# pzou1974/foremast-1

Measured on AMD Instinct MI355X. Metric: metric-series scored/sec (whole node) + p50 detect latency, 100k-series canary, higher is better.
Workload: dtype bf16

## Files before the change

### foremast_amd/ops/csrc/hw_scan.hip

```cpp
#include "common.h"
#include "detect.h"
#include "args.h"

#include <cstdlib>
#include <type_traits>

extern __shared__ __attribute__((aligned(16))) char fm_hw_smem[];

namespace {

enum { MODE_ES = 0, MODE_DES = 1, MODE_HW = 2 };

template <int CTRL, int RM>
__device__ __forceinline__ float dppf(float old, float src) {
  return __int_as_float(__builtin_amdgcn_update_dpp(__float_as_int(old), __float_as_int(src), CTRL, RM, 0xf, false));
}
template <int CTRL, int RM>
__device__ __forceinline__ v2f dpp2(float old, v2f src) {
  v2f r;
  r.x = dppf<CTRL, RM>(old, src.x);
  r.y = dppf<CTRL, RM>(old, src.y);
  return r;
}
__device__ __forceinline__ float rdlane(float v, int l) {
// ... 364 lines not shown
  v2f r;
  r.x = __int_as_float(__builtin_amdgcn_mov_dpp(__float_as_int(src.x), CTRL, RM, 0xf, true));
  r.y = __int_as_float(__builtin_amdgcn_mov_dpp(__float_as_int(src.y), CTRL, RM, 0xf, true));
  return r;
}
template <int CTRL>
__device__ __forceinline__ void row_round_z(v2f& w1, v2f& w2, const Mat2& Bd) {
  const v2f q1 = dppz2<CTRL, 0xf>(w1);
  const v2f q2 = dppz2<CTRL, 0xf>(w2);
  w1 = w1 + Bd.a * q1 + Bd.b * q2;
  w2 = w2 + Bd.c * q1 + Bd.d * q2;
}
__device__ __forceinline__ void half_uniform_scan_pre(const Mat2* Bp, cfp tab_b, v2f v1, v2f v2, v2f x01, v2f x02,
                                                      const Mat2& Bj, bool odd_row, v2f& s1, v2f& s2) {
  const Mat2 B16 = ldmat(tab_b + 32);
  v2f w1 = dppz2<0x111, 0xf>(v1);
  v2f w2 = dppz2<0x111, 0xf>(v2);
  row_round_z<0x111>(w1, w2, Bp[0]);
  row_round_z<0x112>(w1, w2, Bp[1]);
  row_round_z<0x114>(w1, w2, Bp[2]);
  row_round_z<0x118>(w1, w2, Bp[3]);
  v2f e1, e2;
  matvec(Bp[0], w1, w2, e1, e2);
  e1 = e1 + v1;
  e2 = e2 + v2;
  const v2f E1 = dppz2<0x142, 0xa>(e1), E2 = dppz2<0x142, 0xa>(e2);
  v2f y1, y2;
  matvec(B16, x01, x02, y1, y2);
  y1 = odd_row ? y1 + E1 : x01;
  y2 = odd_row ? y2 + E2 : x02;
  matvec(Bj, y1, y2, s1, s2);
  s1 = s1 + w1;
  s2 = s2 + w2;
}

__device__ __forceinline__ void row_uniform_scan_pre(const Mat2* Bp, v2f v1, v2f v2, v2f x01, v2f x02,
                                                     const Mat2& Bj, v2f& s1, v2f& s2) {
  v2f w1 = dppz2<0x111, 0xf>(v1);
  v2f w2 = dppz2<0x111, 0xf>(v2);
  row_round_z<0x111>(w1, w2, Bp[0]);
  row_round_z<0x112>(w1, w2, Bp[1]);
  row_round_z<0x114>(w1, w2, Bp[2]);
  row_round_z<0x118>(w1, w2, Bp[3]);
  matvec(Bj, x01, x02, s1, s2);
  s1 = s1 + w1;
  s2 = s2 + w2;
}

template <typename V>
__device__ __forceinline__ void half_exclusive_scan(Aff<V>& a, int j) {
  scan_round<0x111, 0xf>(a);
  scan_round<0x112, 0xf>(a);
  scan_round<0x114, 0xf>(a);
  scan_round<0x118, 0xf>(a);
  scan_round<0x142, 0xa>(a);
  a.m11 = dppv<0x138, 0xf>(1.f, a.m11);
  a.m12 = dppv<0x138, 0xf>(0.f, a.m12);
  a.m21 = dppv<0x138, 0xf>(0.f, a.m21);
  a.m22 = dppv<0x138, 0xf>(1.f, a.m22);
  a.v1 = dppv<0x138, 0xf>(0.f, a.v1);
  a.v2 = dppv<0x138, 0xf>(0.f, a.v2);
  if (j == 0) {
    const V one = splatv<V>(1.f), zero = splatv<V>(0.f);
    a.m11 = one; a.m12 = zero; a.m21 = zero; a.m22 = one; a.v1 = zero; a.v2 = zero;
  }
}
// ... 344 lines not shown
      "v_add_f32_dpp %0, %0, %0 row_bcast:15 row_mask:0xa bank_mask:0xf\n"
      "v_add_f32_dpp %1, %1, %1 row_bcast:15 row_mask:0xa bank_mask:0xf\n"
      "s_nop 1"
      : "+v"(v.x), "+v"(v.y));
  return v;
}

__device__ __forceinline__ v2f row_sum_last(v2f v) {
  asm volatile(
      "s_nop 1\n"
      "v_add_f32_dpp %0, %0, %0 row_shr:1 row_mask:0xf bank_mask:0xf bound_ctrl:1\n"
      "v_add_f32_dpp %1, %1, %1 row_shr:1 row_mask:0xf bank_mask:0xf bound_ctrl:1\n"
      "s_nop 1\n"
      "v_add_f32_dpp %0, %0, %0 row_shr:2 row_mask:0xf bank_mask:0xf bound_ctrl:1\n"
      "v_add_f32_dpp %1, %1, %1 row_shr:2 row_mask:0xf bank_mask:0xf bound_ctrl:1\n"
      "s_nop 1\n"
      "v_add_f32_dpp %0, %0, %0 row_shr:4 row_mask:0xf bank_mask:0xf bound_ctrl:1\n"
      "v_add_f32_dpp %1, %1, %1 row_shr:4 row_mask:0xf bank_mask:0xf bound_ctrl:1\n"
      "s_nop 1\n"
      "v_add_f32_dpp %0, %0, %0 row_shr:8 row_mask:0xf bank_mask:0xf bound_ctrl:1\n"
      "v_add_f32_dpp %1, %1, %1 row_shr:8 row_mask:0xf bank_mask:0xf bound_ctrl:1\n"
      "s_nop 1"
      : "+v"(v.x), "+v"(v.y));
  return v;
}

template <int SEL>
__device__ __forceinline__ v2f pk_splat(v2f pair) {
  v2f r;
  if (SEL == 0) asm volatile("v_pk_mov_b32 %0, %1, %1 op_sel:[0,0]" : "=v"(r) : "v"(pair));
  else asm volatile("v_pk_mov_b32 %0, %1, %1 op_sel:[1,1]" : "=v"(r) : "v"(pair));
  return r;
}
template <int K, int R>
__device__ __forceinline__ void d_pass1_steps(int q, const Chunk8f& cc, const v2f* wc, v2f* D, v2f& p1, v2f& p2) {
  if constexpr (R < 8) {
    const int i = 8 * q + R;
    if (i < K) {
      D[i] = pk_splat<R & 1>(chunk_pair<R>(cc));
      p1 = p1 + wc[2 * R] * D[i];
      p2 = p2 + wc[2 * R + 1] * D[i];
    }
    d_pass1_steps<K, R + 1>(q, cc, wc, D, p1, p2);
  }
}

template <int K>
__device__ __forceinline__ void d_pass1(const float* blk, cfp W, v2f* D, v2f& p1, v2f& p2) {
  constexpr int NCH = (K + 7) / 8;
  p1 = splat2(0.f);
  p2 = splat2(0.f);
  Chunk8f cc, cn;
  cn.load(blk);
#pragma unroll
  for (int q = 0; q < NCH; ++q) {
    v2f wc[16];
    W = launder(W);
#pragma unroll
    for (int r = 0; r < 16; ++r)
      if (16 * q + r < 2 * K) wc[r] = ldv2(W + 32 * q + 2 * r);
    cc = cn;
    if (q + 1 < NCH) cn.load(blk + (q + 1) * D_CHUNK);
    fence_sched();
    d_pass1_steps<K, 0>(q, cc, wc, D, p1, p2);
    fence_sched();
  }
}

__device__ __forceinline__ v2f keep_if(v2f e, unsigned keep, int bit) {
  const int mk = ((int)(keep << (31 - bit))) >> 31;
  v2f r;
  r.x = __int_as_float(__float_as_int(e.x) & mk);
  r.y = __int_as_float(__float_as_int(e.y) & mk);
  return r;
}

template <int K, bool FUSE, int R, bool M2 = false, bool R1 = false, bool SAVE = false>
__device__ __forceinline__ void d_steps(int q, const Chunk8f& cc, v2f* D, v2f c1, v2f c2, v2f g1a, const v2f* wc,
                                        v2f& x1, v2f& x2, v2f& sse, v2f& p1, v2f& p2, unsigned k2 = 0u,
                                        unsigned k1 = 0u, v2f* E = nullptr) {
  if constexpr (R < 8) {
    const int i = 8 * q + R;
    if (i < K) {
      v2f e = D[i] - x1;
      if (M2) e = keep_if(e, k2, i & 31);
      if constexpr (SAVE) {
        if (i & 1) asm volatile("v_mov_b32 %0, %1" : "=v"(E[i >> 1].y) : "v"(e.x));
        else asm volatile("v_mov_b32 %0, %1" : "=v"(E[i >> 1].x) : "v"(e.x));
      }
      const v2f t = x1 + x2;
      x1 = t + c1 * e;
      x2 = x2 + c2 * e;
      sse = sse + e * e;
      if (FUSE) {
        D[i] = add_dy<R>(D[i], cc) - g1a * e;
        if (R1) {
          const v2f tz = p1 + p2;
          const v2f ez = keep_if(D[i] - p1, k1, i & 31);
          p1 = tz + c1 * ez;
          p2 = p2 + c2 * ez;
        } else {
          p1 = p1 + wc[2 * R] * D[i];
          p2 = p2 + wc[2 * R + 1] * D[i];
        }
      } else if (i < HALF_HB) {
        D[i] = D[i] - g1a * e;
      }
    }
    d_steps<K, FUSE, R + 1, M2, R1, SAVE>(q, cc, D, c1, c2, g1a, wc, x1, x2, sse, p1, p2, k2, k1, E);
  }
}

template <int K>
__device__ __forceinline__ void d_chunk0(const float* blk, cfp W, Chunk8f& c, v2f* w) {
  c.load(blk);
#pragma unroll
  for (int r = 0; r < 16; ++r)
    if (r < 2 * K) w[r] = ldv2(W + 2 * r);
}

template <int K, bool FUSE, bool M2 = false, bool R1 = false, int L = 32, bool SAVE = false>
__device__ __forceinline__ void d_pass2(const float* blk, v2f* D, v2f c1, v2f c2, v2f g1a, cfp W, v2f& x1,
                                        v2f& x2, v2f& sse, v2f& p1, v2f& p2, cfp tb = nullptr,
                                        Mat2* Bn = nullptr, bool chk = false, const unsigned* ubp = nullptr,
                                        int* alive = nullptr, const Chunk8f* c0 = nullptr, const v2f* w0 = nullptr,
                                        unsigned k2lo = 0u, unsigned k2hi = 0u, unsigned k1lo = 0u,
                                        unsigned k1hi = 0u, v2f* E = nullptr) {
  constexpr int NCH = (K + 7) / 8;
  constexpr bool WTS = FUSE && !R1;
  if (FUSE) { p1 = splat2(0.f); p2 = splat2(0.f); }
  fence_sched();
  Chunk8f cc, cn;
  v2f wc[16], wn[16];
  unsigned ub = 0x7f800000u;
  if (FUSE && chk) ub = __hip_atomic_load(ubp, __ATOMIC_RELAXED, __HIP_MEMORY_SCOPE_WORKGROUP);
  if (WTS) {
    if (c0) {
      cn = *c0;
#pragma unroll
      for (int r = 0; r < 16; ++r) wn[r] = w0[r];
    } else {
      d_chunk0<K>(blk, W, cn, wn);
    }
  } else if (FUSE) {
    cn.load(blk);
  }
#pragma unroll
  for (int q = 0; q < NCH; ++q) {
    if (FUSE && q + 1 == NCH && chk) {
      const v2f s = L == 32 ? half_sum_last(sse) : row_sum_last(sse);
      const float U = __uint_as_float(ub);
      int v = ((lane_id() & (L - 1)) == L - 1 && !(s.x > U && s.y > U)) ? 1 : 0;
      asm volatile("" : "+v"(v));
      *alive = v;
    }
    if (WTS) {
      cc = cn;
#pragma unroll
      for (int r = 0; r < 16; ++r) wc[r] = wn[r];
      asm volatile("" ::"v"(cc.lo.x), "v"(cc.hi.x), "s"(wc[0].x));
      if (q + 1 < NCH) {
        W = launder(W);
        cn.load(blk + (q + 1) * D_CHUNK);
#pragma unroll
        for (int r = 0; r < 16; ++r)
          if (16 * (q + 1) + r < 2 * K) wn[r] = ldv2(W + 32 * (q + 1) + 2 * r);
      } else if (Bn) {
        tb = launder(tb);
#pragma unroll
        for (int b = 0; b < 4; ++b) Bn[b] = ldmat(tb + 8 * b);
      }
    } else if (FUSE) {
      cc = cn;
      asm volatile("" ::"v"(cc.lo.x), "v"(cc.hi.x));
      if (q + 1 < NCH) cn.load(blk + (q + 1) * D_CHUNK);
    }
    fence_sched();
    d_steps<K, FUSE, 0, M2, R1, SAVE>(q, cc, D, c1, c2, g1a, wc, x1, x2, sse, p1, p2, q < 4 ? k2lo : k2hi,
                                      q < 4 ? k1lo : k1hi, E);
    fence_sched();
  }
  if (WTS && Bn) {
    asm volatile("" ::"s"(Bn[0].a.x), "s"(Bn[3].d.y));
    fence_sched();
  }
}

__device__ __forceinline__ int hint_pair_at(int k, int lo, unsigned hp) {
  const int h0 = (int)(hp & 0xffffu), h1 = (int)(hp >> 16);
  const int nh = (h0 != 0xffff) + (h1 != 0xffff);
  if (k < nh) return (k == 0 && h0 != 0xffff) ? h0 : h1;
  int r = lo + k - nh;
  const int a0 = h0 < h1 ? h0 : h1, a1 = h0 < h1 ? h1 : h0;
  r += r >= a0 ? 1 : 0;
  r += r >= a1 ? 1 : 0;
  return r;
}

constexpr int QUAD_ITEM = 0x10000;
struct QuadQueue {
  int h0, h1, nh, nq, n_items;
  bool sib;
  __device__ __forceinline__ QuadQueue(int lo, int hi, unsigned hp) {
    h0 = (int)(hp & 0xffffu);
    h1 = (int)(hp >> 16);
    if (h0 == 0xffff) { h0 = h1; h1 = 0xffff; }
    nh = (h0 != 0xffff) + (h1 != 0xffff);
    sib = nh == 2 && (h0 ^ 1) == h1;
    nq = ((hi - lo) >> 1) - (sib ? 1 : nh);
    n_items = nh + nq + (sib ? 0 : nh);
  }
  __device__ __forceinline__ int at(int k, int lo) const {
    if (k < nh) return k == 0 ? h0 : h1;
    k -= nh;
    if (k < nq) {
      int r = (lo >> 1) + k;
      const int q0 = h0 >> 1, q1 = sib ? 0x7fff : h1 >> 1;
      const int a0 = q0 < q1 ? q0 : q1, a1 = q0 < q1 ? q1 : q0;
      r += r >= a0 ? 1 : 0;
      r += r >= a1 ? 1 : 0;
      return (2 * r) | QUAD_ITEM;
    }
    return (k == nq ? h0 : h1) ^ 1;
  }
};

template <int K, int R>
__device__ __forceinline__ void d_replay_steps(int q, const Chunk8f& cd, const Chunk8f& cy, const v2f* wc,
                                               const v2f* E, v2f g1a, v2f* D, v2f& p1, v2f& p2) {
  if constexpr (R < 8) {
    const int i = 8 * q + R;
    if (i < K) {
      D[i] = pk_splat<R & 1>(chunk_pair<R>(cd));
      D[i] = add_dy<R>(D[i], cy) - g1a * pk_splat<R & 1>(E[i >> 1]);
      p1 = p1 + wc[2 * R] * D[i];
      p2 = p2 + wc[2 * R + 1] * D[i];
    }
    d_replay_steps<K, R + 1>(q, cd, cy, wc, E, g1a, D, p1, p2);
  }
}

template <int K>
__device__ __forceinline__ void d_replay(const float* blk, const float* dyb, cfp W, const v2f* E, v2f g1a, v2f* D,
                                         v2f& p1, v2f& p2) {
  constexpr int NCH = (K + 7) / 8;
  p1 = splat2(0.f);
  p2 = splat2(0.f);
  Chunk8f cd, cy;
#pragma unroll
  for (int q = 0; q < NCH; ++q) {
    v2f wc[16];
    W = launder(W);
#pragma unroll
    for (int r = 0; r < 16; ++r)
      if (16 * q + r < 2 * K) wc[r] = ldv2(W + 32 * q + 2 * r);
    cd.load(blk + q * D_CHUNK);
    cy.load(dyb + q * D_CHUNK);
    fence_sched();
    d_replay_steps<K, 0>(q, cd, cy, wc, E, g1a, D, p1, p2);
    fence_sched();
  }
}


template <int K, int S>
struct DLds {
  static constexpr int SEA = DLay<K>::SEASON;
  static constexpr int NMW = ((64 / S) * K + 31) / 32;
  static constexpr int ZEROED = S * NMW + 4 * S * D_WAVES + 4;
  static constexpr int QUEUE = S, HINTS = S + 1;
  static constexpr int UBOUND = (S + 2 + 3) & ~3;
  static constexpr int FIXED = ZEROED + S * HALF_HB + D_WAVES * S * HALF_HB + D_WAVES * S * 4 + UBOUND;
  __host__ __device__ static constexpr size_t words(int ns1) { return (size_t)S * ns1 * SEA + FIXED; }
  __host__ __device__ static constexpr size_t gap_words(int ns1) { return (size_t)2 * ns1 * 64 + 2 * ns1 + 2; }

  float* dl;
  unsigned* vmask;
  float* stat;
  int* flag;
  float* ylast;
  float* bests;
  float* wbest;
  unsigned* ubound;
  unsigned* mbits;
  int* segm;
  float* nvc;
  __device__ __forceinline__ explicit DLds(int ns1) {
    dl = (float*)fm_hw_smem;
    vmask = (unsigned*)(dl + (size_t)S * ns1 * SEA);
    stat = (float*)(vmask + S * NMW);
    flag = (int*)(stat + 4 * S * D_WAVES);
    ylast = (float*)(flag + 4);
// ... 330 lines not shown
      const int q = atomicAdd(deferred, 1);
      if (q < (a.N + 1) / 2) deferred[1 + q] = n0;
    }
    return;
  }
  d_lds_init(L, a, tid, n0, hints, pi_lo, pi_hi);
  const int head = a.head_dev ? *a.head_dev : a.head;
  __syncthreads();

  int bad = 0;
  d_stage<T>(L, a, n0, head, tid, lane, w, bad);
  if (bad) atomicOr(L.flag, 1);
  __syncthreads();
  if (*L.flag) {
    if (tid == 0 && hid == 0) {
      const int q = atomicAdd(deferred, 1);
      if (q < (a.N + 1) / 2) deferred[1 + q] = n0;
      gflags[n0 >> 1] = 1;
    }
    return;
  }
  float l0r[2], b0r[2];
  d_means(L, m, ns1, tid, l0r, b0r);
  __syncthreads();

  const float l0 = pick(l0r, half), b0 = pick(b0r, half);
  const float* mydl = L.dl + (size_t)half * ns1 * SEA + j * 4;
  const int last_addr = ((lane & 32) | 31) << 2;
  Best best = {__builtin_huge_valf(), 0x7fffffff, l0, b0};
  float* mybest = L.bests + (w * 2 + half) * HALF_HB;
  const int nwaves = blockDim.x / FM_WAVE;
  const int npb = pi_hi - pi_lo;
  const unsigned hints_pp = (unsigned)__builtin_amdgcn_readfirstlane((int)L.ubound[L.HINTS]);
  const bool quads = share && ns1 >= 2 && ((pi_lo | pi_hi) & 1) == 0;
  const QuadQueue qq(pi_lo, pi_hi, hints_pp);
  const int n_items = quads ? qq.n_items : npb;
  v2f D[K];
  v2f E[(K + 1) / 2];
  float sX1, sX2, ssse;
  constexpr int ALONE = 0, FIRST = 1, SECOND = 2;
  const auto walk = [&](auto mode, int pi) __attribute__((always_inline)) {
    constexpr int MODE = decltype(mode)::value;
    GridPair<K> gp(a, pi, lane);
    v2f X1, X2, sse, p1, p2;
    if constexpr (MODE == SECOND) {
      d_replay<K>(mydl, mydl + SEA, gp.W, E, gp.g1a, D, p1, p2);
      X1 = splat2(sX1); X2 = splat2(sX2); sse = splat2(ssse);
    } else {
      X1 = splat2(l0 + b0); X2 = splat2(b0); sse = splat2(0.f);
      d_pass1<K>(mydl, gp.W, D, p1, p2);
    }
    if constexpr (MODE == FIRST) {
      v2f x1, x2;
      Chunk8f c0;
      v2f w0[16];
      asm volatile("" : "+v"(sse));
      d_chunk0<K>(mydl + SEA, launder(gp.W), c0, w0);
      half_uniform_scan_pre(gp.Bp, launder(gp.tb), p1, p2, X1, X2, gp.Bj, odd_row, x1, x2);
      d_pass2<K, true, false, false, 32, true>(mydl + SEA, D, gp.c1, gp.c2, gp.g1a, launder(gp.W), x1, x2, sse, p1, p2,
                                               gp.tb, gp.Bp, false, nullptr, nullptr, &c0, w0, 0u, 0u, 0u, 0u, E);
      X1 = half_last_bp(x1, last_addr);
      X2 = half_last_bp(x2, last_addr);
      sX1 = X1.x; sX2 = X2.x; ssse = sse.x;
    }
    int alive = 1;
    for (int sg = MODE == ALONE ? 1 : 2; sg < nseg - 1; ++sg) {
      v2f x1, x2;
      Chunk8f c0;
      v2f w0[16];
      d_chunk0<K>(mydl + (size_t)sg * SEA, launder(gp.W), c0, w0);
      half_uniform_scan_pre(gp.Bp, launder(gp.tb), p1, p2, X1, X2, gp.Bj, odd_row, x1, x2);
      d_pass2<K, true>(mydl + (size_t)sg * SEA, D, gp.c1, gp.c2, gp.g1a, launder(gp.W), x1, x2, sse, p1, p2, gp.tb,
                       gp.Bp, PRUNE, L.ubound + half, &alive, &c0, w0);
      X1 = half_last_bp(x1, last_addr);
      X2 = half_last_bp(x2, last_addr);
      if (PRUNE && !__any(alive)) break;
    }
    if (!PRUNE || __any(alive)) {
      v2f x1, x2, d1, d2;
      half_uniform_scan_pre(gp.Bp, gp.tb, p1, p2, X1, X2, gp.Bj, odd_row, x1, x2);
      d_pass2<K, false>(mydl, D, gp.c1, gp.c2, gp.g1a, gp.W, x1, x2, sse, d1, d2);
      X1 = half_last_bp(x1, last_addr);
      X2 = half_last_bp(x2, last_addr);
      sse = half_sum_last(sse);
      sse = half_last_bp(sse, last_addr);
      take_candidate<PRUNE>(best, sse, X1, X2, gp.c0, gp.c1i, j == 0, L.ubound + half,
                            [&](bool upd1) __attribute__((always_inline)) {
        first_lane_phases<K>(mybest, L.ylast + half * HALF_HB, D, upd1, j, hmax);
      });
    }
  };
  for (int k = w; k < n_items;) {
    const int item = quads ? qq.at(k, pi_lo) : hint_pair_at(k, pi_lo, hints_pp);
    if (item & QUAD_ITEM) {
      walk(std::integral_constant<int, FIRST>(), item & 0xffff);
      walk(std::integral_constant<int, SECOND>(), (item & 0xffff) + 1);
    } else {
      walk(std::integral_constant<int, ALONE>(), item);
    }
    k = queue_pop(L.ubound + L.QUEUE, lane, nwaves);
  }

  if (j == 0) put_wave_best<2>(L.wbest, w, half, best);
  __syncthreads();
  if (w >= 2) return;
  const int r = w, n = n0 + r;
  if (n >= a.N) return;
  const int win = wave_argmin<2>(L.wbest, r, nwaves);
  const float* wb = L.wbest + (win * 2 + r) * 4;
  float gSSE = wb[0], gL = wb[2], gB = wb[3];
  int gIdx = __float_as_int(wb[1]);
  float* sb = L.bests + (win * 2 + r) * HALF_HB;
  if (slot >= 0) {
    float* mine = cand + (((size_t)slot * 2 + hid) * 2 + r) * CAND_FLOATS;
    if (lane < HALF_HB) __hip_atomic_store(&mine[4 + lane], sb[lane], __ATOMIC_RELAXED, __HIP_MEMORY_SCOPE_SYSTEM);
    if (lane == 0) {
      __hip_atomic_store(&mine[0], gSSE, __ATOMIC_RELAXED, __HIP_MEMORY_SCOPE_SYSTEM);
      __hip_atomic_store(&mine[1], __int_as_float(gIdx), __ATOMIC_RELAXED, __HIP_MEMORY_SCOPE_SYSTEM);
      __hip_atomic_store(&mine[2], gL, __ATOMIC_RELAXED, __HIP_MEMORY_SCOPE_SYSTEM);
      __hip_atomic_store(&mine[3], gB, __ATOMIC_RELAXED, __HIP_MEMORY_SCOPE_SYSTEM);
    }
    asm volatile("s_waitcnt vmcnt(0)" ::: "memory");
    int prev = 0;
    if (lane == 0) prev = __hip_atomic_fetch_add(&cnt[slot * 2 + r], 1, __ATOMIC_RELAXED, __HIP_MEMORY_SCOPE_AGENT);
    prev = __shfl(prev, 0, FM_WAVE);
    if (prev == 0) return;
    if (lane == 0) __hip_atomic_store(&cnt[slot * 2 + r], 0, __ATOMIC_RELAXED, __HIP_MEMORY_SCOPE_AGENT);
    const float* oth = cand + (((size_t)slot * 2 + (1 - hid)) * 2 + r) * CAND_FLOATS;
    const float oSSE = __hip_atomic_load(&oth[0], __ATOMIC_RELAXED, __HIP_MEMORY_SCOPE_SYSTEM);
    const int oIdx = __float_as_int(__hip_atomic_load(&oth[1], __ATOMIC_RELAXED, __HIP_MEMORY_SCOPE_AGENT));
    if (oSSE < gSSE || (oSSE == gSSE && oIdx < gIdx)) {
      gSSE = oSSE;
      gIdx = oIdx;
// ... 562 lines not shown
static bool d_supported_k(int K) { return K == 45 || K == 9; }
static bool q_supported_k(int K) { return K == 18; }

static size_t d_lds_words(int Tp, int seg, int K, bool gapped) {
  if (!d_supported_k(K) || seg <= 0) return (size_t)-1;
  const int nseg = Tp / seg;
  if (nseg < 2 || nseg > D_MAXSEG) return (size_t)-1;
  const int ns1 = nseg - 1;
  const size_t gap = gapped ? DLds<45, 2>::gap_words(ns1) : 0;
  return (K == 45 ? DLds<45, 2>::words(ns1) : DLds<9, 2>::words(ns1)) + gap;
}

extern "C" size_t fm_hw_d_lds_bytes(int Tp, int seg, int K) {
  const size_t words = d_lds_words(Tp, seg, K, false);
  return words == (size_t)-1 ? words : words * 4;
}

extern "C" size_t fm_hw_dg_lds_bytes(int Tp, int seg, int K) {
  const size_t words = d_lds_words(Tp, seg, K, true);
  return words == (size_t)-1 ? words : words * 4;
}

extern "C" size_t fm_hw_q_lds_bytes(int Tp, int seg, int K) {
  if (!q_supported_k(K) || seg != 16 * K) return (size_t)-1;
  const int nseg = Tp / seg;
  if (nseg < 2 || nseg > D_MAXSEG) return (size_t)-1;
  return DLds<18, Q_S>::words(nseg - 1) * 4;
}

struct GridSwitches {
  bool prune;
  int hints;
  int share;
};
static GridSwitches grid_switches() {
  const char* pe = getenv("FOREMAST_HW_PRUNE");
  const char* he = getenv("FOREMAST_HW_HINTS");
  const char* se = getenv("FOREMAST_HW_SHARE");
  GridSwitches s;
  s.prune = !(pe && pe[0] == '0');
  s.hints = (s.prune && !(he && he[0] == '0')) ? 1 : 0;
  s.share = !(se && se[0] == '0') ? 1 : 0;
  return s;
}

template <bool PRUNE, typename T>
static hipError_t launch_q_fit(const SmoothArgs* a, const float* tab_g, int hmax, int* deferred, int hints,
                               hipStream_t st) {
  const int K = a->K;
  const size_t lds = fm_hw_q_lds_bytes(a->Tp, a->seg, K);
  const size_t dlds = fm_hw_dg_lds_bytes(a->Tp, a->seg, K / 2);
  const int quads = (a->N + 3) / 4;
  hipLaunchKernelGGL((hw_q_kernel<18, PRUNE, T>), dim3(quads), dim3(256), lds, st, *a, hmax, deferred, hints);
  hipError_t e = hipGetLastError();
  if (e != hipSuccess) return e;
  SmoothArgs ag = *a;
  ag.pair_tab = tab_g;
  ag.K = K / 2;
  const int pairs = (a->N + 1) / 2;
  const int grid = pairs < 512 ? pairs : 512;
  hipLaunchKernelGGL((hw_dg_kernel<9, PRUNE, T>), dim3(grid), dim3(256), dlds, st, ag, hmax, deferred, hints);
  return hipGetLastError();
}

extern "C" int fm_hw_q_fit_dt(const SmoothArgs* a, const float* tab_g, int hmax, int* deferred, hipStream_t st,
                              int fp32) {
  const int K = a->K;
  if (!q_supported_k(K) || a->seg != 16 * K || a->m != a->seg || a->Tp % a->seg != 0 || a->Tp / a->seg < 2 ||
      a->Tp / a->seg > D_MAXSEG || !a->pair_tab || !tab_g || a->season_out || hmax < 1 || hmax > K ||
      hmax > HALF_HB)
    return (int)hipErrorNotSupported;
  if (a->N <= 0) return 0;
  if (fm_hw_q_lds_bytes(a->Tp, a->seg, K) > 80 * 1024 || fm_hw_dg_lds_bytes(a->Tp, a->seg, K / 2) > 80 * 1024)
    return (int)hipErrorNotSupported;
  if (!deferred) return (int)hipErrorInvalidValue;
// ... 93 lines not shown
  if (e != hipSuccess) return e;
  const char* ge = getenv("FOREMAST_HW_GAPS");
  if (K == 45 && std::is_same<T, bf16_t>::value && ge && ge[0] == 'v') {
    const size_t glds = fm_hw_half_lds_bytes(a->Tp, a->seg, K);
    if (glds > 64 * 1024) return hipErrorNotSupported;
    hipLaunchKernelGGL((hw_half_general_kernel<45>), dim3(pairs < 512 ? pairs : 512), dim3(256), glds, st, *a, hmax,
                       deferred);
    return hipGetLastError();
  }
  const size_t dlds = fm_hw_dg_lds_bytes(a->Tp, a->seg, K);
  int grid = pairs < 512 ? pairs : 512;
  const char* gg = getenv("FOREMAST_HW_DG_GRID");
  if (gg && atoi(gg) > 0) grid = atoi(gg) < pairs ? atoi(gg) : pairs;
  hipLaunchKernelGGL((hw_dg_kernel<K, PRUNE, T>), dim3(grid), dim3(256), dlds, st, *a, hmax, deferred, hints);
  return hipGetLastError();
}

extern "C" int fm_hw_d_fit_split_dt(const SmoothArgs* a, int hmax, int* deferred, int* split_ws, int max_split,
                                    int slots, hipStream_t st, int grid_quads, int fp32) {
  const int K = a->K;
  if (!d_supported_k(K) || a->seg != 32 * K || a->m != a->seg || a->Tp % a->seg != 0 || a->Tp / a->seg < 2 ||
      a->Tp / a->seg > D_MAXSEG || !a->pair_tab || a->season_out || hmax < 1 || hmax > K || hmax > HALF_HB)
    return (int)hipErrorNotSupported;
  if (a->N <= 0) return 0;
  if (fm_hw_d_lds_bytes(a->Tp, a->seg, K) > 80 * 1024 || fm_hw_dg_lds_bytes(a->Tp, a->seg, K) > 80 * 1024)
    return (int)hipErrorNotSupported;
  if (!deferred) return (int)hipErrorInvalidValue;
  const GridSwitches sw = grid_switches();
  const auto launch =
      fp32 ? (K == 45 ? (sw.prune ? launch_d_fit<45, true, float> : launch_d_fit<45, false, float>)
                      : (sw.prune ? launch_d_fit<9, true, float> : launch_d_fit<9, false, float>))
           : (K == 45 ? (sw.prune ? launch_d_fit<45, true, bf16_t> : launch_d_fit<45, false, bf16_t>)
                      : (sw.prune ? launch_d_fit<9, true, bf16_t> : launch_d_fit<9, false, bf16_t>));
  return (int)launch(a, hmax, deferred, split_ws, max_split, slots, sw.hints, (sw.share && grid_quads) ? 1 : 0, st);
}

extern "C" int fm_hw_d_fit_split(const SmoothArgs* a, int hmax, int* deferred, int* split_ws, int max_split,
                                 int slots, hipStream_t st, int grid_quads) {
  return fm_hw_d_fit_split_dt(a, hmax, deferred, split_ws, max_split, slots, st, grid_quads, 0);
}

extern "C" int fm_hw_d_fit(const SmoothArgs* a, int hmax, int* deferred, hipStream_t st) {
  return fm_hw_d_fit_split(a, hmax, deferred, nullptr, 0, 0, st, 0);
}

template <int K, int MODE, typename TIN, int NC, int MINW, bool TAB = false>
__global__ __launch_bounds__(256, MINW) void hw_scan_kernel(const SmoothArgs a) {
  static_assert(!TAB || NC == 2, "table path is packed-pair only");
  using V = typename std::conditional<NC == 2, v2f, float>::type;
  using YR = YRegs<TIN, K>;
  constexpr int KP = YR::KP;
  const int n = blockIdx.x;
  const int tid = threadIdx.x, lane = lane_id(), w = wave_id();
  const int nwaves = blockDim.x / FM_WAVE;
  const int seg = a.seg;
  const int L = seg / K;
  const int nseg = a.Tp / seg;

  size_t off = 0;
  TIN* ys = (TIN*)(fm_hw_smem + off);
  off += ((size_t)nseg * 64 * KP * sizeof(TIN) + 15) & ~(size_t)15;
  float* bests = (float*)(fm_hw_smem + off);
  if (MODE == MODE_HW) off += (size_t)nwaves * 64 * KP * 4;
  int* segnan = (int*)(fm_hw_smem + off);
  off += ((size_t)nseg * 4 + 15) & ~(size_t)15;
  float* red = (float*)(fm_hw_smem + off);
  off += 64 * 4;
// ... 300 lines not shown
```

### foremast_amd/ops/kernels.py

```python

from __future__ import annotations

import collections
import ctypes as C
import os
from dataclasses import dataclass
from typing import Tuple, Dict, Optional

import torch

from . import _native as nat

MODE_ES, MODE_DES, MODE_HW = 0, 1, 2
DEFAULT_ES_K = 16
LDS_LIMIT = 64 * 1024
D_LDS_LIMIT = 78 * 1024
LDS_MAX_WG = 160 * 1024


class KernelShapeError(ValueError):
    pass


def _need(cond: bool, msg: str) -> None:
# ... 257 lines not shown
            c1 = al + c2
            A = np.array([[1 - c1, 1.0], [-c2, 1.0]])
            Ap = np.eye(2)
            for n in range(K + 1):
                for q, v in enumerate((Ap[0, 0], Ap[0, 1], Ap[1, 0], Ap[1, 1])):
                    pw[p, n, 2 * q + comp] = v
                Ap = A @ Ap
    t = torch.tensor(np.concatenate([tab.reshape(-1), pw.reshape(-1)]), dtype=torch.float32,
                     device=grid.device).contiguous()
    if len(_PAIR_TAB_CACHE) > 64:
        _PAIR_TAB_CACHE.clear()
    _PAIR_TAB_CACHE[key] = t
    return t


_GRID_QUADS_CACHE: Dict[tuple, bool] = {}


def grid_has_quads(grid: torch.Tensor) -> bool:
    key = (grid.data_ptr(), tuple(grid.shape), grid.device)
    hit = _GRID_QUADS_CACHE.get(key)
    if hit is None:
        G = grid.shape[0]
        hit = False
        if G > 0 and G % 4 == 0 and grid.dim() == 2 and grid.shape[1] >= 2:
            ab = grid.detach()[:, :2].float().cpu().contiguous().view(torch.int32).view(G // 4, 4, 2)
            hit = bool((ab == ab[:, :1]).all())
        if len(_GRID_QUADS_CACHE) > 64:
            _GRID_QUADS_CACHE.clear()
        _GRID_QUADS_CACHE[key] = hit
    return hit


def smoothing_supported(mode: int, T: int, m: int, bf16: bool) -> bool:
    try:
        Tp, _, k, seg = smoothing_geometry(mode, T, m)
    except KernelShapeError:
        return False
    lib = nat.load()
    if lib is None:
        return False
    return lib.fm_smooth_lds_bytes(Tp, m if mode == MODE_HW else 1, seg, int(bf16)) <= LDS_LIMIT


def _fit_outputs(out: Optional[Dict[str, torch.Tensor]], N: int, dev, names, m: int = 0,
                 zeroed=()) -> Dict[str, torch.Tensor]:
    out = {} if out is None else out
    for name in names:
        if name not in out:
            shape = (N, HALF_HB) if name == "season_hb" else (N, m) if name == "season" else (N,)
            make = torch.zeros if name in zeroed else torch.empty
            out[name] = make(shape, dtype=torch.int32 if name == "best" else torch.float32, device=dev)
    return out


def _smooth_args(out: Dict[str, torch.Tensor], N: int, *, Tp: int, m: int, pad: int = 0, K: int = 0, seg: int = 0,
                 hist: Optional[torch.Tensor] = None, head: int = 0, length: int = 0,
                 grid: Optional[torch.Tensor] = None) -> "nat.SmoothArgs":
    a = nat.SmoothArgs()
    if hist is not None:
        a.hist = nat.ptr(hist)
        a.ld = hist.stride(0)
        a.ring_len = hist.shape[1]
        a.head = int(head)
        a.T = int(length)
    a.Tp, a.pad, a.m, a.K, a.seg = int(Tp), int(pad), int(m), int(K), int(seg)
# ... 133 lines not shown
    N = hist.shape[0]
    k = m // 16 if quad else m // 32
    out = _fit_outputs(out, N, dev, ("level", "trend", "sigma", "best") + (("season_hb", "nvalid") if defer else ()))
    a = _smooth_args(out, N, Tp=Tp, m=m, pad=pad, K=k, seg=m, hist=hist, head=head, length=length, grid=grid)
    a.pair_tab = nat.ptr(pair_table(grid, k))
    if head_dev is not None:
        _need(head_dev.dtype == torch.int32 and head_dev.device == dev and head_dev.numel() >= 1,
              "head_dev must be an int32 device scalar")
        a.head_dev = nat.ptr(head_dev)
    _fill_detect(a.det, det, N, dev, out)
    _set_hvar(a.det, det, grid, MODE_HW, m)
    if defer:
        a.season_hb = nat.ptr(out["season_hb"])
        a.nvalid_out = nat.ptr(out["nvalid"])
        a.det.C = 0
    ws = _half_workspace(dev, N)
    global last_hw_variant, last_detect_deferred
    last_detect_deferred = defer
    fp32 = int(hist.dtype == torch.float32)
    _need(residual or not fp32, "HW variant 4 needs a bfloat16 ring")
    if quad:
        rc = lib.fm_hw_q_fit_dt(a, nat.ptr(pair_table(grid, m // 32)), int(hmax), nat.ptr(ws),
                                nat.stream_handle(dev), fp32)
        if rc != 0:
            ws.zero_()
        nat.check(rc, "fm_hw_q_fit_dt")
        last_hw_variant = 5
        return out
    if residual:
        sws, slots = _split_workspace(dev)
        if os.environ.get("FOREMAST_HW_SPLIT", "1") == "0":
            slots = 0
        rc = lib.fm_hw_d_fit_split_dt(a, int(hmax), nat.ptr(ws), nat.ptr(sws), SPLIT_MAX, slots,
                                      nat.stream_handle(dev), int(grid_has_quads(grid)), fp32)
        if rc != 0:
            ws.zero_()
        nat.check(rc, "fm_hw_d_fit_split_dt")
        last_hw_variant = 5
        return out
    rc = lib.fm_hw_half_fit(a, int(hmax), nat.ptr(ws), nat.stream_handle(dev))
    if rc != 0:
        ws.zero_()
    nat.check(rc, "fm_hw_half_fit")
    last_hw_variant = 4
    return out


def _hw_seq_fit(lib, hist, head, length, m, grid, det, Tp, pad, out, want_season: bool,
                head_dev: Optional[torch.Tensor] = None, defer: bool = False, detect_after=None):
    dev = hist.device
    N = hist.shape[0]
    out = _fit_outputs(out, N, dev, ("level", "trend", "sigma", "nvalid", "best", "season_hb")
                       + (("season",) if want_season else ()), m=m)
    if not defer and detect_after is not None:
        torch.cuda.current_stream(dev).wait_stream(detect_after)
    a = _smooth_args(out, N, Tp=Tp, m=m, pad=pad, K=1, seg=m, hist=hist, head=head, length=length, grid=grid)
    a.season_out = nat.ptr(out["season"]) if want_season else 0
    a.nvalid_out = nat.ptr(out["nvalid"])
    a.season_hb = nat.ptr(out["season_hb"])
    if head_dev is not None:
        _need(head_dev.dtype == torch.int32 and head_dev.device == dev and head_dev.numel() >= 1,
              "head_dev must be an int32 device scalar")
        a.head_dev = nat.ptr(head_dev)
    _fill_detect(a.det, det, N, dev, out)
    _set_hvar(a.det, det, grid, MODE_HW, m)
    if defer:
        a.det.C = 0
# ... 1014 lines not shown
```

Before: 11.69 million.

## Add level-only fast path for zero-beta grid quads in Holt-Winters fit

```diff
diff --git a/foremast_amd/ops/csrc/hw_scan.hip b/foremast_amd/ops/csrc/hw_scan.hip
--- a/foremast_amd/ops/csrc/hw_scan.hip
+++ b/foremast_amd/ops/csrc/hw_scan.hip
@@ -420,6 +420,28 @@
   matvec(Bj, y1, y2, s1, s2);
   s1 = s1 + w1;
   s2 = s2 + w2;
+}
+
+template <int CTRL>
+__device__ __forceinline__ void row_round_z1(v2f& w1, v2f a) {
+  const v2f q1 = dppz2<CTRL, 0xf>(w1);
+  w1 = w1 + a * q1;
+}
+__device__ __forceinline__ void half_uniform_scan_pre_level(const Mat2* Bp, cfp tab_b, v2f v1, v2f x01, v2f x02,
+                                                            const Mat2& Bj, bool odd_row, v2f& s1) {
+  const v2f B16a = ldv2(tab_b + 32), B16b = ldv2(tab_b + 34);
+  v2f w1 = dppz2<0x111, 0xf>(v1);
+  row_round_z1<0x111>(w1, Bp[0].a);
+  row_round_z1<0x112>(w1, Bp[1].a);
+  row_round_z1<0x114>(w1, Bp[2].a);
+  row_round_z1<0x118>(w1, Bp[3].a);
+  v2f e1 = Bp[0].a * w1;
+  e1 = e1 + v1;
+  const v2f E1 = dppz2<0x142, 0xa>(e1);
+  v2f y1 = B16a * x01 + B16b * x02;
+  y1 = odd_row ? y1 + E1 : x01;
+  s1 = Bj.a * y1 + Bj.b * x02;
+  s1 = s1 + w1;
 }
 
 __device__ __forceinline__ void row_uniform_scan_pre(const Mat2* Bp, v2f v1, v2f v2, v2f x01, v2f x02,
@@ -830,20 +852,20 @@
   else asm volatile("v_pk_mov_b32 %0, %1, %1 op_sel:[1,1]" : "=v"(r) : "v"(pair));
   return r;
 }
-template <int K, int R>
+template <int K, int R, bool LV = false>
 __device__ __forceinline__ void d_pass1_steps(int q, const Chunk8f& cc, const v2f* wc, v2f* D, v2f& p1, v2f& p2) {
   if constexpr (R < 8) {
     const int i = 8 * q + R;
     if (i < K) {
       D[i] = pk_splat<R & 1>(chunk_pair<R>(cc));
       p1 = p1 + wc[2 * R] * D[i];
-      p2 = p2 + wc[2 * R + 1] * D[i];
-    }
-    d_pass1_steps<K, R + 1>(q, cc, wc, D, p1, p2);
-  }
-}
-
-template <int K>
+      if constexpr (!LV) p2 = p2 + wc[2 * R + 1] * D[i];
+    }
+    d_pass1_steps<K, R + 1, LV>(q, cc, wc, D, p1, p2);
+  }
+}
+
+template <int K, bool LV = false>
 __device__ __forceinline__ void d_pass1(const float* blk, cfp W, v2f* D, v2f& p1, v2f& p2) {
   constexpr int NCH = (K + 7) / 8;
   p1 = splat2(0.f);
@@ -856,11 +878,11 @@
     W = launder(W);
 #pragma unroll
     for (int r = 0; r < 16; ++r)
-      if (16 * q + r < 2 * K) wc[r] = ldv2(W + 32 * q + 2 * r);
+      if (16 * q + r < 2 * K && !(LV && (r & 1))) wc[r] = ldv2(W + 32 * q + 2 * r);
     cc = cn;
     if (q + 1 < NCH) cn.load(blk + (q + 1) * D_CHUNK);
     fence_sched();
-    d_pass1_steps<K, 0>(q, cc, wc, D, p1, p2);
+    d_pass1_steps<K, 0, LV>(q, cc, wc, D, p1, p2);
     fence_sched();
   }
 }
@@ -873,7 +895,7 @@
   return r;
 }
 
-template <int K, bool FUSE, int R, bool M2 = false, bool R1 = false, bool SAVE = false>
+template <int K, bool FUSE, int R, bool M2 = false, bool R1 = false, bool SAVE = false, bool LV = false>
 __device__ __forceinline__ void d_steps(int q, const Chunk8f& cc, v2f* D, v2f c1, v2f c2, v2f g1a, const v2f* wc,
                                         v2f& x1, v2f& x2, v2f& sse, v2f& p1, v2f& p2, unsigned k2 = 0u,
                                         unsigned k1 = 0u, v2f* E = nullptr) {
@@ -888,7 +910,7 @@
       }
       const v2f t = x1 + x2;
       x1 = t + c1 * e;
-      x2 = x2 + c2 * e;
+      if constexpr (!LV) x2 = x2 + c2 * e;
       sse = sse + e * e;
       if (FUSE) {
         D[i] = add_dy<R>(D[i], cc) - g1a * e;
@@ -899,25 +921,25 @@
           p2 = p2 + c2 * ez;
         } else {
           p1 = p1 + wc[2 * R] * D[i];
-          p2 = p2 + wc[2 * R + 1] * D[i];
+          if constexpr (!LV) p2 = p2 + wc[2 * R + 1] * D[i];
         }
       } else if (i < HALF_HB) {
         D[i] = D[i] - g1a * e;
       }
     }
-    d_steps<K, FUSE, R + 1, M2, R1, SAVE>(q, cc, D, c1, c2, g1a, wc, x1, x2, sse, p1, p2, k2, k1, E);
-  }
-}
-
-template <int K>
+    d_steps<K, FUSE, R + 1, M2, R1, SAVE, LV>(q, cc, D, c1, c2, g1a, wc, x1, x2, sse, p1, p2, k2, k1, E);
+  }
+}
+
+template <int K, bool LV = false>
 __device__ __forceinline__ void d_chunk0(const float* blk, cfp W, Chunk8f& c, v2f* w) {
   c.load(blk);
 #pragma unroll
   for (int r = 0; r < 16; ++r)
-    if (r < 2 * K) w[r] = ldv2(W + 2 * r);
-}
-
-template <int K, bool FUSE, bool M2 = false, bool R1 = false, int L = 32, bool SAVE = false>
+    if (r < 2 * K && !(LV && (r & 1))) w[r] = ldv2(W + 2 * r);
+}
+
+template <int K, bool FUSE, bool M2 = false, bool R1 = false, int L = 32, bool SAVE = false, bool LV = false>
 __device__ __forceinline__ void d_pass2(const float* blk, v2f* D, v2f c1, v2f c2, v2f g1a, cfp W, v2f& x1,
                                         v2f& x2, v2f& sse, v2f& p1, v2f& p2, cfp tb = nullptr,
                                         Mat2* Bn = nullptr, bool chk = false, const unsigned* ubp = nullptr,
@@ -936,9 +958,10 @@
     if (c0) {
       cn = *c0;
 #pragma unroll
-      for (int r = 0; r < 16; ++r) wn[r] = w0[r];
+      for (int r = 0; r < 16; ++r)
+        if (!(LV && (r & 1))) wn[r] = w0[r];
     } else {
-      d_chunk0<K>(blk, W, cn, wn);
+      d_chunk0<K, LV>(blk, W, cn, wn);
     }
   } else if (FUSE) {
     cn.load(blk);
@@ -955,18 +978,22 @@
     if (WTS) {
       cc = cn;
 #pragma unroll
-      for (int r = 0; r < 16; ++r) wc[r] = wn[r];
+      for (int r = 0; r < 16; ++r)
+        if (!(LV && (r & 1))) wc[r] = wn[r];
       asm volatile("" ::"v"(cc.lo.x), "v"(cc.hi.x), "s"(wc[0].x));
       if (q + 1 < NCH) {
         W = launder(W);
         cn.load(blk + (q + 1) * D_CHUNK);
 #pragma unroll
         for (int r = 0; r < 16; ++r)
-          if (16 * (q + 1) + r < 2 * K) wn[r] = ldv2(W + 32 * (q + 1) + 2 * r);
+          if (16 * (q + 1) + r < 2 * K && !(LV && (r & 1))) wn[r] = ldv2(W + 32 * (q + 1) + 2 * r);
       } else if (Bn) {
         tb = launder(tb);
 #pragma unroll
-        for (int b = 0; b < 4; ++b) Bn[b] = ldmat(tb + 8 * b);
+        for (int b = 0; b < 4; ++b) {
+          if constexpr (LV) Bn[b].a = ldv2(tb + 8 * b);
+          else Bn[b] = ldmat(tb + 8 * b);
+        }
       }
     } else if (FUSE) {
       cc = cn;
@@ -974,12 +1001,13 @@
       if (q + 1 < NCH) cn.load(blk + (q + 1) * D_CHUNK);
     }
     fence_sched();
-    d_steps<K, FUSE, 0, M2, R1, SAVE>(q, cc, D, c1, c2, g1a, wc, x1, x2, sse, p1, p2, q < 4 ? k2lo : k2hi,
-                                      q < 4 ? k1lo : k1hi, E);
+    d_steps<K, FUSE, 0, M2, R1, SAVE, LV>(q, cc, D, c1, c2, g1a, wc, x1, x2, sse, p1, p2, q < 4 ? k2lo : k2hi,
+                                          q < 4 ? k1lo : k1hi, E);
     fence_sched();
   }
   if (WTS && Bn) {
-    asm volatile("" ::"s"(Bn[0].a.x), "s"(Bn[3].d.y));
+    if constexpr (LV) asm volatile("" ::"s"(Bn[0].a.x), "s"(Bn[3].a.y));
+    else asm volatile("" ::"s"(Bn[0].a.x), "s"(Bn[3].d.y));
     fence_sched();
   }
 }
@@ -1023,7 +1051,7 @@
   }
 };
 
-template <int K, int R>
+template <int K, int R, bool LV = false>
 __device__ __forceinline__ void d_replay_steps(int q, const Chunk8f& cd, const Chunk8f& cy, const v2f* wc,
                                                const v2f* E, v2f g1a, v2f* D, v2f& p1, v2f& p2) {
   if constexpr (R < 8) {
@@ -1032,13 +1060,13 @@
       D[i] = pk_splat<R & 1>(chunk_pair<R>(cd));
       D[i] = add_dy<R>(D[i], cy) - g1a * pk_splat<R & 1>(E[i >> 1]);
       p1 = p1 + wc[2 * R] * D[i];
-      p2 = p2 + wc[2 * R + 1] * D[i];
-    }
-    d_replay_steps<K, R + 1>(q, cd, cy, wc, E, g1a, D, p1, p2);
-  }
-}
-
-template <int K>
+      if constexpr (!LV) p2 = p2 + wc[2 * R + 1] * D[i];
+    }
+    d_replay_steps<K, R + 1, LV>(q, cd, cy, wc, E, g1a, D, p1, p2);
+  }
+}
+
+template <int K, bool LV = false>
 __device__ __forceinline__ void d_replay(const float* blk, const float* dyb, cfp W, const v2f* E, v2f g1a, v2f* D,
                                          v2f& p1, v2f& p2) {
   constexpr int NCH = (K + 7) / 8;
@@ -1051,11 +1079,11 @@
     W = launder(W);
 #pragma unroll
     for (int r = 0; r < 16; ++r)
-      if (16 * q + r < 2 * K) wc[r] = ldv2(W + 32 * q + 2 * r);
+      if (16 * q + r < 2 * K && !(LV && (r & 1))) wc[r] = ldv2(W + 32 * q + 2 * r);
     cd.load(blk + q * D_CHUNK);
     cy.load(dyb + q * D_CHUNK);
     fence_sched();
-    d_replay_steps<K, 0>(q, cd, cy, wc, E, g1a, D, p1, p2);
+    d_replay_steps<K, 0, LV>(q, cd, cy, wc, E, g1a, D, p1, p2);
     fence_sched();
   }
 }
@@ -1452,35 +1480,42 @@
   const int nwaves = blockDim.x / FM_WAVE;
   const int npb = pi_hi - pi_lo;
   const unsigned hints_pp = (unsigned)__builtin_amdgcn_readfirstlane((int)L.ubound[L.HINTS]);
-  const bool quads = share && ns1 >= 2 && ((pi_lo | pi_hi) & 1) == 0;
+  const bool quads = (share & 1) && ns1 >= 2 && ((pi_lo | pi_hi) & 1) == 0;
   const QuadQueue qq(pi_lo, pi_hi, hints_pp);
   const int n_items = quads ? qq.n_items : npb;
   v2f D[K];
   v2f E[(K + 1) / 2];
   float sX1, sX2, ssse;
   constexpr int ALONE = 0, FIRST = 1, SECOND = 2;
-  const auto walk = [&](auto mode, int pi) __attribute__((always_inline)) {
+  const auto walk = [&](auto mode, auto level, int pi) __attribute__((always_inline)) -> bool {
     constexpr int MODE = decltype(mode)::value;
+    constexpr bool LV = decltype(level)::value;
     GridPair<K> gp(a, pi, lane);
     v2f X1, X2, sse, p1, p2;
     if constexpr (MODE == SECOND) {
-      d_replay<K>(mydl, mydl + SEA, gp.W, E, gp.g1a, D, p1, p2);
+      d_replay<K, LV>(mydl, mydl + SEA, gp.W, E, gp.g1a, D, p1, p2);
       X1 = splat2(sX1); X2 = splat2(sX2); sse = splat2(ssse);
     } else {
       X1 = splat2(l0 + b0); X2 = splat2(b0); sse = splat2(0.f);
-      d_pass1<K>(mydl, gp.W, D, p1, p2);
+      d_pass1<K, LV>(mydl, gp.W, D, p1, p2);
     }
     if constexpr (MODE == FIRST) {
       v2f x1, x2;
       Chunk8f c0;
       v2f w0[16];
       asm volatile("" : "+v"(sse));
-      d_chunk0<K>(mydl + SEA, launder(gp.W), c0, w0);
-      half_uniform_scan_pre(gp.Bp, launder(gp.tb), p1, p2, X1, X2, gp.Bj, odd_row, x1, x2);
-      d_pass2<K, true, false, false, 32, true>(mydl + SEA, D, gp.c1, gp.c2, gp.g1a, launder(gp.W), x1, x2, sse, p1, p2,
-                                               gp.tb, gp.Bp, false, nullptr, nullptr, &c0, w0, 0u, 0u, 0u, 0u, E);
+      d_chunk0<K, LV>(mydl + SEA, launder(gp.W), c0, w0);
+      if constexpr (LV) {
+        half_uniform_scan_pre_level(gp.Bp, launder(gp.tb), p1, X1, X2, gp.Bj, odd_row, x1);
+        x2 = X2;
+      } else {
+        half_uniform_scan_pre(gp.Bp, launder(gp.tb), p1, p2, X1, X2, gp.Bj, odd_row, x1, x2);
+      }
+      d_pass2<K, true, false, false, 32, true, LV>(mydl + SEA, D, gp.c1, gp.c2, gp.g1a, launder(gp.W), x1, x2, sse, p1,
+                                                   p2, gp.tb, gp.Bp, false, nullptr, nullptr, &c0, w0, 0u, 0u, 0u, 0u,
+                                                   E);
       X1 = half_last_bp(x1, last_addr);
-      X2 = half_last_bp(x2, last_addr);
+      if constexpr (!LV) X2 = half_last_bp(x2, last_addr);
       sX1 = X1.x; sX2 = X2.x; ssse = sse.x;
     }
     int alive = 1;
@@ -1488,20 +1523,35 @@
       v2f x1, x2;
       Chunk8f c0;
       v2f w0[16];
-      d_chunk0<K>(mydl + (size_t)sg * SEA, launder(gp.W), c0, w0);
-      half_uniform_scan_pre(gp.Bp, launder(gp.tb), p1, p2, X1, X2, gp.Bj, odd_row, x1, x2);
-      d_pass2<K, true>(mydl + (size_t)sg * SEA, D, gp.c1, gp.c2, gp.g1a, launder(gp.W), x1, x2, sse, p1, p2, gp.tb,
-                       gp.Bp, PRUNE, L.ubound + half, &alive, &c0, w0);
+      d_chunk0<K, LV>(mydl + (size_t)sg * SEA, launder(gp.W), c0, w0);
+      if constexpr (LV) {
+        half_uniform_scan_pre_level(gp.Bp, launder(gp.tb), p1, X1, X2, gp.Bj, odd_row, x1);
+        x2 = X2;
+      } else {
+        half_uniform_scan_pre(gp.Bp, launder(gp.tb), p1, p2, X1, X2, gp.Bj, odd_row, x1, x2);
+      }
+      d_pass2<K, true, false, false, 32, false, LV>(mydl + (size_t)sg * SEA, D, gp.c1, gp.c2, gp.g1a, launder(gp.W), x1,
+                                                    x2, sse, p1, p2, gp.tb, gp.Bp, PRUNE, L.ubound + half, &alive, &c0,
+                                                    w0);
       X1 = half_last_bp(x1, last_addr);
-      X2 = half_last_bp(x2, last_addr);
+      if constexpr (!LV) X2 = half_last_bp(x2, last_addr);
       if (PRUNE && !__any(alive)) break;
     }
     if (!PRUNE || __any(alive)) {
       v2f x1, x2, d1, d2;
-      half_uniform_scan_pre(gp.Bp, gp.tb, p1, p2, X1, X2, gp.Bj, odd_row, x1, x2);
-      d_pass2<K, false>(mydl, D, gp.c1, gp.c2, gp.g1a, gp.W, x1, x2, sse, d1, d2);
+      if constexpr (LV) {
+        half_uniform_scan_pre_level(gp.Bp, gp.tb, p1, X1, X2, gp.Bj, odd_row, x1);
+        x2 = X2;
+      } else {
+        half_uniform_scan_pre(gp.Bp, gp.tb, p1, p2, X1, X2, gp.Bj, odd_row, x1, x2);
+      }
+      d_pass2<K, false, false, false, 32, false, LV>(mydl, D, gp.c1, gp.c2, gp.g1a, gp.W, x1, x2, sse, d1, d2);
       X1 = half_last_bp(x1, last_addr);
-      X2 = half_last_bp(x2, last_addr);
+      if constexpr (!LV) X2 = half_last_bp(x2, last_addr);
+      if constexpr (LV) {
+        const unsigned ex = 0x7f800000u;
+        if (__any((__float_as_uint(X1.x) & ex) == ex || (__float_as_uint(X1.y) & ex) == ex)) return true;
+      }
       sse = half_sum_last(sse);
       sse = half_last_bp(sse, last_addr);
       take_candidate<PRUNE>(best, sse, X1, X2, gp.c0, gp.c1i, j == 0, L.ubound + half,
@@ -1509,16 +1559,32 @@
         first_lane_phases<K>(mybest, L.ylast + half * HALF_HB, D, upd1, j, hmax);
       });
     }
+    return false;
   };
-  for (int k = w; k < n_items;) {
-    const int item = quads ? qq.at(k, pi_lo) : hint_pair_at(k, pi_lo, hints_pp);
+  const unsigned level = (unsigned)share >> 1;
+  int redo = -1;
+  for (int k = w; k < n_items || redo >= 0;) {
+    int item;
+    if (redo >= 0) {
+      item = redo & 0xffff;
+      redo = (redo & QUAD_ITEM) ? (item ^ 1) : -1;
+    } else {
+      item = quads ? qq.at(k, pi_lo) : hint_pair_at(k, pi_lo, hints_pp);
+    }
     if (item & QUAD_ITEM) {
-      walk(std::integral_constant<int, FIRST>(), item & 0xffff);
-      walk(std::integral_constant<int, SECOND>(), (item & 0xffff) + 1);
+      const int pf = item & 0xffff;
+      if (pf < 32 && ((level >> (pf >> 1)) & 1u)) {
+        const bool r0 = walk(std::integral_constant<int, FIRST>(), std::true_type(), pf);
+        const bool r1 = walk(std::integral_constant<int, SECOND>(), std::true_type(), pf + 1);
+        if (r0 || r1) redo = (r0 ? pf : pf + 1) | ((r0 && r1) ? QUAD_ITEM : 0);
+      } else {
+        walk(std::integral_constant<int, FIRST>(), std::false_type(), pf);
+        walk(std::integral_constant<int, SECOND>(), std::false_type(), pf + 1);
+      }
     } else {
-      walk(std::integral_constant<int, ALONE>(), item);
-    }
-    k = queue_pop(L.ubound + L.QUEUE, lane, nwaves);
+      walk(std::integral_constant<int, ALONE>(), std::false_type(), item);
+    }
+    if (redo < 0) k = queue_pop(L.ubound + L.QUEUE, lane, nwaves);
   }
 
   if (j == 0) put_wave_best<2>(L.wbest, w, half, best);
@@ -2147,6 +2213,7 @@
   bool prune;
   int hints;
   int share;
+  int level;
 };
 static GridSwitches grid_switches() {
   const char* pe = getenv("FOREMAST_HW_PRUNE");
@@ -2156,6 +2223,8 @@
   s.prune = !(pe && pe[0] == '0');
   s.hints = (s.prune && !(he && he[0] == '0')) ? 1 : 0;
   s.share = !(se && se[0] == '0') ? 1 : 0;
+  const char* le = getenv("FOREMAST_HW_LEVEL");
+  s.level = !(le && le[0] == '0') ? 1 : 0;
   return s;
 }
 
@@ -2315,7 +2384,8 @@
                       : (sw.prune ? launch_d_fit<9, true, float> : launch_d_fit<9, false, float>))
            : (K == 45 ? (sw.prune ? launch_d_fit<45, true, bf16_t> : launch_d_fit<45, false, bf16_t>)
                       : (sw.prune ? launch_d_fit<9, true, bf16_t> : launch_d_fit<9, false, bf16_t>));
-  return (int)launch(a, hmax, deferred, split_ws, max_split, slots, sw.hints, (sw.share && grid_quads) ? 1 : 0, st);
+  const int share = (sw.share && (grid_quads & 1)) ? (1 | (sw.level ? (grid_quads & 0x1fffe) : 0)) : 0;
+  return (int)launch(a, hmax, deferred, split_ws, max_split, slots, sw.hints, share, st);
 }
 
 extern "C" int fm_hw_d_fit_split(const SmoothArgs* a, int hmax, int* deferred, int* split_ws, int max_split,
diff --git a/foremast_amd/ops/kernels.py b/foremast_amd/ops/kernels.py
--- a/foremast_amd/ops/kernels.py
+++ b/foremast_amd/ops/kernels.py
@@ -313,6 +313,27 @@
     return hit
 
 
+_GRID_LEVEL_CACHE: Dict[tuple, int] = {}
+
+
+def grid_level_mask(grid: torch.Tensor) -> int:
+    if os.environ.get("FOREMAST_HW_LEVEL", "1")[:1] == "0":
+        return 0
+    key = (grid.data_ptr(), tuple(grid.shape), grid.device)
+    hit = _GRID_LEVEL_CACHE.get(key)
+    if hit is None:
+        hit = 0
+        if grid_has_quads(grid):
+            G = grid.shape[0]
+            beta = grid.detach()[:, 1].float().cpu().contiguous().view(torch.int32).view(G // 4, 4)
+            zero = (beta == 0).all(dim=1).tolist()
+            hit = sum(1 << q for q, z in enumerate(zero[:16]) if z)
+        if len(_GRID_LEVEL_CACHE) > 64:
+            _GRID_LEVEL_CACHE.clear()
+        _GRID_LEVEL_CACHE[key] = hit
+    return hit
+
+
 def smoothing_supported(mode: int, T: int, m: int, bf16: bool) -> bool:
     try:
         Tp, _, k, seg = smoothing_geometry(mode, T, m)
@@ -512,7 +533,8 @@
         if os.environ.get("FOREMAST_HW_SPLIT", "1") == "0":
             slots = 0
         rc = lib.fm_hw_d_fit_split_dt(a, int(hmax), nat.ptr(ws), nat.ptr(sws), SPLIT_MAX, slots,
-                                      nat.stream_handle(dev), int(grid_has_quads(grid)), fp32)
+                                      nat.stream_handle(dev),
+                                      int(grid_has_quads(grid)) | (grid_level_mask(grid) << 1), fp32)
         if rc != 0:
             ws.zero_()
         nat.check(rc, "fm_hw_d_fit_split_dt")
```

Result: no change. 11.80 million (median of 6 runs) (+0.9%).
